# doubiliu/bellman-mpc

Measured on AMD Instinct MI355X. Metric: Groth16 constraints/sec, BLS12-381, 2^22-constraint R1CS, higher is better.
Workload: dtype u32 limbs (BLS12-381 Fp/Fr modular integer)

## Files before the change

bellman-mpc_amd/csrc/msm.h:

```cpp
#pragma once
#include <hip/hip_runtime.h>
#include <stddef.h>
#include <stdint.h>

#include <mutex>

#include "curve.cuh"
#include "kinfo.h"

namespace bh {

constexpr uint32_t G1_TABLE_REC = 32;

struct MsmShape {
  int c;
  int W;
  int NB;
  int L;
  int S;
  int Wb;
  int pre;
  int rec;
  uint32_t bk_lo = 0, bk_hi = 0;
  bool bucket_shard() const { return bk_hi > bk_lo; }
  uint32_t red_lo() const { return bucket_shard() ? bk_lo : 0u; }
  uint32_t red_nb() const { return bucket_shard() ? bk_hi - bk_lo : (uint32_t)NB; }
};
constexpr uint32_t BUCKET_SHARD_GRANULE = 1024;
MsmShape msm_shape(size_t n, int c_override);
int msm_table_c(size_t n);
MsmShape msm_shape_table(size_t n, int c);

uint32_t reduce_block_max(bool g2);
inline uint32_t reduce_threads_for(uint32_t nbr, uint32_t L, bool g2) {
  const uint32_t T = nbr / L, bmax = reduce_block_max(g2);
  return T < bmax ? T : bmax;
}
inline uint32_t reduce_block_threads(const MsmShape& sh, bool g2) {
  return reduce_threads_for((uint32_t)sh.NB, (uint32_t)sh.L, g2);
}
inline int reduce_lg2(uint32_t x) {
  int r = 0;
  while ((1u << r) < x) r++;
  return r;
}
inline int reduce_shift_for(uint32_t nbr, uint32_t L, bool g2) {
  return reduce_lg2(L) + reduce_lg2(reduce_threads_for(nbr, L, g2));
}
inline int reduce_split_shift(const MsmShape& sh, bool g2) {
  return sh.Wb == 1 ? reduce_shift_for(sh.red_nb(), (uint32_t)sh.L, g2) : -1;
}
inline void reduce_level2(uint32_t nblk, bool g2, uint32_t* BT2, uint32_t* Lb) {
  const uint32_t bmax = g2 ? 128u : 256u;
  uint32_t lb = 1;
  while ((size_t)bmax * lb < nblk) lb <<= 1;
  uint32_t t = 1;
  while ((size_t)t * lb < nblk) t <<= 1;
  *BT2 = t;
  *Lb = lb;
}

struct MsmTiming {
  hipEvent_t ev_acc_begin = nullptr, ev_acc_end = nullptr;
};

constexpr uint32_t G2_TABLE_REC = 64;

template <class C>
struct MsmWorkspace {
  size_t cap_n = 0, cap_E = 0, cap_nbt = 0, cap_segs = 0, cap_T = 0;
  uint32_t *entries = nullptr, *counts = nullptr, *offsets = nullptr, *cursor = nullptr, *scan_scratch = nullptr,
           *cont_bucket = nullptr, *tilecounts = nullptr, *tscan = nullptr;
  uint2* recs = nullptr;
  size_t cap_tc = 0;
  typename C::P *bucket_sums = nullptr, *conts = nullptr, *seg_weighted = nullptr, *seg_sum = nullptr,
                *window_sums = nullptr;
// ... 21 lines not shown
template <class C>
hipError_t msm_accumulate(MsmWorkspace<C>& ws, hipStream_t st, const uint32_t* d_bases, size_t n, const MsmShape& sh,
                          MsmTiming* timing);
template <class C>
hipError_t msm_front(MsmWorkspace<C>& ws, hipStream_t st, const uint32_t* d_bases, const uint32_t* d_scalars,
                     size_t n, const int32_t* d_idx, uint32_t base_offset, const MsmShape& sh, MsmTiming* timing);
template <class C>
hipError_t msm_back(MsmWorkspace<C>& ws, hipStream_t st, size_t n, const MsmShape& sh, typename C::P* host_out,
                    int max_span = -1, hipEvent_t acc_done = nullptr, const uint32_t* d_span_words = nullptr);

size_t scan_scratch_words(size_t n);
template <class C>
void msm_acc_kernels(std::vector<KernInfo>& v);
template <class C>
void msm_back_kernels(std::vector<KernInfo>& v);
size_t reduce_blocks_resident_per_cu_g1();
constexpr uint32_t MAX_SPAN_BLOCKS = 256;
inline uint32_t max_span_blocks(size_t nbt) {
  const size_t g = (nbt + 255) / 256;
  return (uint32_t)(g < 1 ? 1 : (g > MAX_SPAN_BLOCKS ? MAX_SPAN_BLOCKS : g));
}
inline uint32_t max_span_host(const uint32_t* h_words, size_t nbt) {
  uint32_t m = 0;
  for (uint32_t b = 0, g = max_span_blocks(nbt); b < g; b++) m = h_words[b] > m ? h_words[b] : m;
  return m;
}
hipError_t max_span(const uint32_t* counts, const uint32_t* offsets, size_t nbt, uint32_t S, uint32_t* d_words,
                    uint32_t* h_words, hipStream_t st);
void exclusive_scan(const uint32_t* in, uint32_t* out, size_t n, uint32_t* scratch, hipStream_t st);
hipError_t scalars_prepare(const uint32_t* d_in, uint32_t* d_out, size_t n, int mode, int log_perm, hipStream_t st);
hipError_t density_index(const uint64_t* d_words, size_t n, uint32_t base_offset, int32_t* d_idx, uint32_t* d_tmp,
// ... 16 lines not shown
```

bellman-mpc_amd/csrc/msm_common.hip:

```cpp
#include "msm.h"

#include <algorithm>

namespace bh {

static inline unsigned blocks_for(size_t n, unsigned bs) { return (unsigned)((n + bs - 1) / bs); }


__device__ __forceinline__ size_t scan_len(size_t n, const uint32_t* dn) {
  return dn ? min(n, (size_t)*dn + 1) : n;
}
__global__ void __launch_bounds__(256) k_scan_tile(const uint32_t* in, uint32_t* out, uint32_t* tile_sums, size_t n,
                                                   const uint32_t* dn) {
  __shared__ uint32_t s[256];
  n = scan_len(n, dn);
  if ((size_t)blockIdx.x * 1024 >= n) {
    if (threadIdx.x == 0 && tile_sums) tile_sums[blockIdx.x] = 0;
    return;
  }
  const size_t base = (size_t)blockIdx.x * 1024 + threadIdx.x * 4;
  uint32_t v[4];
  uint32_t local = 0;
#pragma unroll
  for (int i = 0; i < 4; i++) {
// ... 132 lines not shown
  if (d > half) {
    carry = 1;
    return (int)d - (int)(1u << c);
  }
  carry = 0;
  return (int)d;
}

__device__ __forceinline__ void load_scalar(const uint32_t* scalars, size_t i, uint32_t* s) {
  const uint4* p = reinterpret_cast<const uint4*>(scalars + i * 8);
  uint4 a = p[0], b = p[1];
  s[0] = a.x; s[1] = a.y; s[2] = a.z; s[3] = a.w;
  s[4] = b.x; s[5] = b.y; s[6] = b.z; s[7] = b.w;
}

static constexpr size_t REDUCE_T_MIN = 16384;

MsmShape msm_shape(size_t n, int c_override) {
  MsmShape sh;
  int c = c_override;
  if (c <= 0) {
    int lg = 0;
    while (((size_t)1 << (lg + 1)) <= n) lg++;
    int c0 = std::max(4, std::min(16, lg - 6));
    int best = c0, best_fill = -1;
    for (int cc = std::max(4, c0 - 1); cc <= std::min(16, c0 + 1); cc++) {
      const int W = (256 + cc - 1) / cc;
      const int top = 256 - (W - 1) * cc;
      const int fill = top * 16 / cc;
      if (fill > best_fill || (fill == best_fill && cc == c0)) { best = cc; best_fill = fill; }
    }
    c = best;
  }
  sh.c = c;
  sh.W = (256 + c - 1) / c;
  sh.NB = 1 << (c - 1);
  sh.L = std::min<int>(8, sh.NB);
  while (sh.L > 1 && (size_t)sh.W * (size_t)(sh.NB / sh.L) < REDUCE_T_MIN) sh.L >>= 1;
  size_t E = n * (size_t)sh.W;
  int S = 16;
  while (S < 256 && E / (size_t)(2 * S) >= ((size_t)1 << 18)) S <<= 1;
  sh.S = S;
  sh.Wb = sh.W;
  sh.pre = 0;
  sh.rec = 0;
  return sh;
}

uint32_t reduce_block_max(bool g2) { return g2 ? 128u : 256u; }

size_t seg_entries(size_t n, size_t used, int W) {
  (void)used;
  return std::max<size_t>(n, 1) * (size_t)std::max(W, 1);
// ... 3 lines not shown
  int best = 16;
  double best_cost = 1e300;
  for (int c = 8; c <= 24; c++) {
    const int W = (256 + c - 1) / c;
    if (255 - (W - 1) * c < 10) continue;
    const double cost = (double)n * W + 6.5 * (double)((size_t)1 << (c - 1));
    if (cost < best_cost) { best_cost = cost; best = c; }
  }
  return best;
}

MsmShape msm_shape_table(size_t n, int c) {
  MsmShape sh = msm_shape(n, c);
  sh.Wb = 1;
  sh.pre = 1;
  while (sh.L > 1 && (size_t)(sh.NB / sh.L) < REDUCE_T_MIN) sh.L >>= 1;
  return sh;
}

static constexpr int PT_TILE = 4096;

__global__ void __launch_bounds__(256) k_part_count(const uint32_t* scalars, size_t n, const int32_t* idx,
                                                    DigitCfg cfg, int lo_bits, uint32_t P, uint32_t ntiles,
                                                    uint32_t plo, uint32_t phi, uint32_t* tilecounts) {
  extern __shared__ uint32_t hist[];
  for (uint32_t i = threadIdx.x; i < P; i += 256) hist[i] = 0;
  __syncthreads();
  const size_t s0 = (size_t)blockIdx.x * PT_TILE;
  const size_t s1 = min(s0 + PT_TILE, n);
  for (size_t s = s0 + threadIdx.x; s < s1; s += 256) {
    if (idx && idx[s] < 0) continue;
// ... 232 lines not shown
  return e;
}

hipError_t density_index(const uint64_t* d_words, size_t n, uint32_t base_offset, int32_t* d_idx, uint32_t* d_tmp,
                         uint32_t* d_scan_scratch, hipStream_t st) {
  const size_t nwords = (n + 63) / 64;
  if (nwords == 0) return hipSuccess;
  hipLaunchKernelGGL(k_density_popc, dim3(blocks_for(nwords, 256)), dim3(256), 0, st, d_words, nwords, d_tmp);
  exclusive_scan(d_tmp, d_tmp, nwords, d_scan_scratch, st);
  hipLaunchKernelGGL(k_density_index, dim3(blocks_for(n, 256)), dim3(256), 0, st, d_words, d_tmp, n, base_offset,
                     d_idx);
  return hipGetLastError();
}

}
```

bellman-mpc_amd/csrc/msm_g1_back.hip:

```cpp
#include "msm_impl.cuh"

namespace bh {
extern template struct MsmWorkspace<G1Ops>;
extern template void fit_segments<G1Ops>(MsmShape&, size_t);
extern template void fit_segments_E<G1Ops>(MsmShape&, size_t);
extern template hipError_t msm_sort<G1Ops>(MsmWorkspace<G1Ops>&, hipStream_t, const uint32_t*, size_t, const int32_t*,
                                            uint32_t, const MsmShape&);
extern template hipError_t msm_accumulate<G1Ops>(MsmWorkspace<G1Ops>&, hipStream_t, const uint32_t*, size_t,
                                                  const MsmShape&, MsmTiming*);

template hipError_t msm_window_sums<G1Ops>(MsmWorkspace<G1Ops>&, hipStream_t, const uint32_t*, const uint32_t*, size_t,
                                         const int32_t*, uint32_t, const MsmShape&, MsmTiming*);
template hipError_t msm_front<G1Ops>(MsmWorkspace<G1Ops>&, hipStream_t, const uint32_t*, const uint32_t*, size_t,
                                   const int32_t*, uint32_t, const MsmShape&, MsmTiming*);
template hipError_t msm_back<G1Ops>(MsmWorkspace<G1Ops>&, hipStream_t, size_t, const MsmShape&, typename G1Ops::P*, int, hipEvent_t, const uint32_t*);
template void msm_back_kernels<G1Ops>(std::vector<KernInfo>&);

size_t reduce_blocks_resident_per_cu_g1() {
  int blocks = 1;
  const int BT = (int)reduce_block_max(false);
  if (hipOccupancyMaxActiveBlocksPerMultiprocessor(&blocks, (const void*)k_reduce_blocks<G1Ops>, BT,
                                                   BT * sizeof(typename G1Ops::P)) != hipSuccess ||
      blocks < 1)
    blocks = 1;
  return (size_t)blocks * BT;
}
}
```

bellman-mpc_amd/csrc/msm_impl.cuh:

```cuda
#pragma once
#include <cstdlib>

#include "msm.h"
#include <algorithm>


namespace bh {

static inline unsigned msm_blocks_for(size_t n, unsigned bs) { return (unsigned)((n + bs - 1) / bs); }

template <class C>
__device__ __forceinline__ void store_point(typename C::P* dst, const typename C::P& p) {
  constexpr int WORDS = sizeof(typename C::P) / 16;
  const uint4* s = reinterpret_cast<const uint4*>(&p);
  uint4* d = reinterpret_cast<uint4*>(dst);
#pragma unroll
  for (int k = 0; k < WORDS; k++) d[k] = s[k];
}
template <class C>
__device__ __forceinline__ typename C::P load_point(const typename C::P* src) {
  typename C::P p;
  constexpr int WORDS = sizeof(typename C::P) / 16;
  const uint4* s = reinterpret_cast<const uint4*>(src);
  uint4* d = reinterpret_cast<uint4*>(&p);
// ... 149 lines not shown
      if (tid == 0) store_point<C>(&conts[s_first + 1], acc);
      __syncthreads();
    }
  }
}


template <class C>
__device__ __forceinline__ typename C::P dbl_times(typename C::P v, int k) {
  for (int j = 0; j < k; j++) v = C::dbl(v);
  return v;
}

template <class C>
__device__ __forceinline__ void block_epilogue(typename C::P v, const typename C::P& base, int lg1,
                                               const typename C::P& extra, int lg2, bool split, typename C::P* lds,
                                               typename C::P* s_blk) {
  const uint32_t i = threadIdx.x, BT = blockDim.x;
  int lgBT = 0;
  while ((1u << lgBT) < BT) lgBT++;
  const int n_final = lg2 >= 0 ? 2 : 1;
  store_point<C>(&lds[i], v);
  __syncthreads();
  const int steps = 2 * lgBT + n_final;
  for (int st = 0; st < steps; st++) {
    typename C::P a = v, b;
    bool act;
    uint32_t dst = i;
    if (st < lgBT) {
      const uint32_t d = 1u << st;
      act = i + d < BT;
      if (act) b = load_point<C>(&lds[i + d]);
    } else if (st < lgBT + n_final) {
      const bool first = st == lgBT;
      if (first) {
        b = i + 1 < BT ? load_point<C>(&lds[i + 1]) : C::identity();
        if (i == 0) *s_blk = load_point<C>(&lds[0]);
      } else {
        b = v;
      }
      b = dbl_times<C>(b, first ? lg1 : lg2);
      a = first ? base : extra;
      act = true;
    } else {
      const uint32_t h = BT >> (st - lgBT - n_final + 1);
      act = split ? i < 2 * h : i < h;
      if (act) {
        dst = i < h ? i : BT + (i - h);
        a = load_point<C>(&lds[dst]);
        b = load_point<C>(&lds[dst + h]);
      }
    }
    __syncthreads();
    if (act) {
      v = C::add(a, b);
      store_point<C>(&lds[dst], v);
    }
    if (split && st == lgBT + n_final - 1) store_point<C>(&lds[BT + i], extra);
    __syncthreads();
  }
}

template <class C>
__global__ void __launch_bounds__(256) k_reduce_blocks(const uint32_t* counts, const uint32_t* offsets,
                                                       const typename C::P* bucket_sums, const typename C::P* conts,
                                                       uint32_t S, uint32_t b0, uint32_t NB, uint32_t L, int lgL,
                                                       uint32_t nblk, int fold, typename C::P* Y, typename C::P* Ssum,
                                                       const uint32_t* span_words, uint32_t span_g, uint32_t fold_span) {
  extern __shared__ uint4 lds_raw[];
  typename C::P* lds = reinterpret_cast<typename C::P*>(lds_raw);
  if (span_words) fold = block_span(span_words, span_g) <= fold_span ? 1 : 0;
  const uint32_t i = threadIdx.x;
  const uint32_t w = blockIdx.x / nblk, blk = blockIdx.x % nblk;
  const uint32_t gb0 = b0 + w * NB + (blk * blockDim.x + i) * L;
  constexpr bool acc_lds = sizeof(typename C::P) > 256;
  typename C::P run = C::identity(), acc = C::identity(), bk = C::identity();
  if (acc_lds) store_point<C>(&lds[i], acc);
  int k = (int)L - 1;
  uint32_t op = 0, c_next = 0, c_end = 0;
  while (k >= 0) {
    typename C::P a, b;
    if (op == 0) {
      const uint32_t gb = gb0 + (uint32_t)k, cnt = counts[gb];
      bk = C::identity();
      c_next = c_end = 0;
      if (cnt) {
        bk = load_point<C>(&bucket_sums[gb]);
        const uint32_t off = offsets[gb];
        const uint32_t s_first = off / S, s_last = (off + cnt - 1) / S;
        c_next = s_first + 1;
        c_end = s_last > s_first ? (fold ? s_last + 1 : s_first + 2) : c_next;
      }
      op = c_next < c_end ? 1 : 2;
      continue;
    }
    if (op == 1) { a = bk; b = load_point<C>(&conts[c_next]); }
    else if (op == 2) { a = run; b = bk; }
    else { a = acc_lds ? load_point<C>(&lds[i]) : acc; b = run; }
    const typename C::P r = C::add(a, b);
    if (op == 1) {
      bk = r;
      if (++c_next == c_end) op = 2;
    } else if (op == 2) {
      run = r;
      op = 3;
    } else {
      if (acc_lds) store_point<C>(&lds[i], r);
      else acc = r;
      op = 0;
      k--;
    }
  }
  if (acc_lds) acc = load_point<C>(&lds[i]);
  __syncthreads();
  typename C::P s_blk;
  block_epilogue<C>(run, acc, lgL, acc, -1, false, lds, &s_blk);
  if (i == 0) {
    store_point<C>(&Y[blockIdx.x], load_point<C>(&lds[0]));
    store_point<C>(&Ssum[blockIdx.x], s_blk);
  }
}

template <class C>
__global__ void __launch_bounds__(256) k_reduce_window(const typename C::P* Y, const typename C::P* Ssum,
                                                       uint32_t nblk, uint32_t Lb, int lgLb, int lgM, int split,
                                                       typename C::P* out) {
  extern __shared__ uint4 lds_raw[];
  typename C::P* lds = reinterpret_cast<typename C::P*>(lds_raw);
  const uint32_t i = threadIdx.x, w = blockIdx.x;
  const size_t base = (size_t)w * nblk + (size_t)i * Lb;
  typename C::P run = C::identity(), acc = C::identity(), p = C::identity();
  for (uint32_t it = 0; it < 3 * Lb; it++) {
    const uint32_t k = Lb - 1 - it / 3, op = it % 3;
    const bool in = i * Lb + k < nblk;
    typename C::P a, b;
    if (op == 0) { a = acc; b = run; }
    else if (op == 1) { a = run; b = in ? load_point<C>(&Ssum[base + k]) : C::identity(); }
    else { a = p; b = in ? load_point<C>(&Y[base + k]) : C::identity(); }
    const typename C::P r = C::add(a, b);
    if (op == 0) acc = r;
    else if (op == 1) run = r;
    else p = r;
  }
  typename C::P s_all;
  block_epilogue<C>(run, acc, lgLb, p, split ? -1 : lgM, split != 0, lds, &s_all);
  if (i == 0) {
    if (split) {
      out[0] = C::reduce(load_point<C>(&lds[blockDim.x]));
      out[1] = C::reduce(load_point<C>(&lds[0]));
      out[2] = C::reduce(s_all);
    } else {
      out[w] = C::reduce(load_point<C>(&lds[0]));
    }
  }
}

#define G2_SB() __builtin_amdgcn_sched_barrier(0)
template <class F, int NW, int NQ, bool ZZ_LDS, bool DIRECT = false, class Issue>
__device__ __forceinline__ void accumulate_lds(uint4 (*pre)[64], int lane, int nq, bool limbs,
                                               const uint32_t* entries, const uint32_t* offsets, uint32_t start,
                                               uint32_t end, uint32_t pos0, uint32_t seg, uint32_t b, uint32_t next,
                                               bool started_here, uint32_t e_cur, uint32_t e_next, Issue& issue,
                                               XYZZ<F>* bucket_sums, XYZZ<F>* conts,
                                               const uint32_t* bases = nullptr, uint32_t rec = 0) {
  using T = typename F::T;
  using Cv = CurveOps<F>;
  constexpr int VW = (NW % 4 == 0) ? 4 : 2;
  constexpr int RH = NW / VW;
// ... 311 lines not shown
    if (hipOccupancyMaxActiveBlocksPerMultiprocessor(&blocks, k, 256, 0) != hipSuccess || blocks < 1) blocks = 1;
    return (size_t)cus * (size_t)blocks * 256;
  }();
  constexpr size_t ROUNDS = 3, MIN_S = 8;
  const size_t slots = std::max<size_t>(ROUNDS * conc / 256 * 256, 256);
  size_t S = (E + slots - 1) / slots;
  sh.S = (int)std::min<size_t>(std::max<size_t>(S, MIN_S), (size_t)1 << 16);
}

template <class C>
size_t MsmWorkspace<C>::bytes_needed(size_t n) {
  MsmShape sh = msm_shape(n, 0);
  size_t E = n * (size_t)sh.W;
  size_t nbt = (size_t)sh.Wb * sh.NB;
  size_t segs = (E + sh.S - 1) / sh.S + 1;
  size_t T = (size_t)sh.Wb * (sh.NB / sh.L);
  return E * 4 + nbt * 4 * 3 + 16 + nbt * sizeof(typename C::P) + segs * sizeof(typename C::P) +
         2 * T * sizeof(typename C::P) + n * 4;
}

template <class C>
hipError_t MsmWorkspace<C>::grow(size_t E, size_t nbt, size_t segs, size_t T) {
  hipError_t err;
  if (E > cap_E) {
    if (entries) hipFree(entries);
    if (recs) hipFree(recs);
    entries = nullptr;
    recs = nullptr;
    if ((err = hipMalloc(&entries, std::max<size_t>(E, 1) * 4)) != hipSuccess) return err;
    if ((err = hipMalloc(&recs, std::max<size_t>(E, 1) * 8)) != hipSuccess) return err;
    cap_E = E;
// ... 31 lines not shown
    cap_T = T;
  }
  if (!window_sums) {
    if ((err = hipMalloc(&window_sums, 256 * sizeof(typename C::P))) != hipSuccess) return err;
    if ((err = hipHostMalloc(&host_window_sums, 256 * sizeof(typename C::P), hipHostMallocDefault)) != hipSuccess)
      return err;
  }
  return hipSuccess;
}

template <class C>
hipError_t MsmWorkspace<C>::reserve_shape(size_t n, const MsmShape& sh) {
  const size_t E = n * (size_t)sh.W;
  const size_t nbt = (size_t)sh.Wb * sh.NB;
  const size_t segs = (E + sh.S - 1) / sh.S + 1;
  const size_t T = (size_t)sh.Wb * (sh.NB / sh.L);
  const size_t tc = sort_tilecount_words(sh, n);
  if (tc > cap_tc) {
    if (tilecounts) hipFree(tilecounts);
    if (tscan) hipFree(tscan);
    tilecounts = tscan = nullptr;
    hipError_t err;
    if ((err = hipMalloc(&tilecounts, tc * 4)) != hipSuccess) return err;
    if ((err = hipMalloc(&tscan, scan_scratch_words(tc) * 4 + 64)) != hipSuccess) return err;
    cap_tc = tc;
  }
  return grow(E, nbt, segs, T);
}

template <class C>
hipError_t MsmWorkspace<C>::reserve(size_t n_max) {
// ... 93 lines not shown
};

struct AccView {
  const uint32_t *counts, *offsets;
  uint32_t S;
  size_t E;
  const uint32_t* span_words;
};
template <class C>
AccView acc_view(const MsmWorkspace<C>& ws, size_t n, const MsmShape& sh) {
  return AccView{ws.counts, ws.offsets, (uint32_t)sh.S, n * (size_t)sh.W, nullptr};
}

template <class C>
static void reduce_range(MsmWorkspace<C>& ws, const AccView& v, hipStream_t st, const MsmShape& sh, size_t segs,
                         size_t span, bool fold, bool seq, uint32_t b0, uint32_t nbr, uint32_t L, uint32_t y_off,
                         typename C::P* out, const SpanSrc& dev = SpanSrc()) {
  constexpr bool G2 = sizeof(typename C::P) > 256;
  const size_t nb_all = (size_t)sh.Wb * nbr;
  const size_t nbt = (size_t)sh.Wb * sh.NB;
  if (dev.words || (!fold && seq)) {
    constexpr int Q = 4;
    constexpr uint32_t B = G2 ? 128 : 256;
    if (dev.words || span >= 2)
      hipLaunchKernelGGL((k_cont_seq<C, Q>), dim3(msm_blocks_for(nb_all * Q, B)), dim3(B), B * sizeof(typename C::P),
                         st, v.counts, v.offsets, b0, (uint32_t)nb_all, v.S, ws.conts, dev.words, dev.g,
                         dev.fold_span, dev.seq_max);
    if (dev.words)
      hipLaunchKernelGGL((k_cont_long<C>), dim3(std::min<unsigned>(msm_blocks_for(nb_all, B), 256u)), dim3(B),
                         B * sizeof(typename C::P), st, v.counts, v.offsets, b0, (uint32_t)nb_all, v.S, ws.conts,
                         dev.words, dev.g, dev.seq_max);
  } else if (!fold) {
    for (size_t stride = 1; stride < span; stride *= 4)
      hipLaunchKernelGGL((k_cont_treeF<C, 4>), dim3(msm_blocks_for(segs, 256)), dim3(256), 0, st, ws.cont_bucket,
                         v.counts, v.offsets, (uint32_t)nbt, v.S, (uint32_t)stride, b0, (uint32_t)(b0 + nb_all),
                         ws.conts);
  }
  const uint32_t T = nbr / L;
  const uint32_t BT = reduce_threads_for(nbr, L, G2);
  const uint32_t nblk = T / BT;
  uint32_t BT2, Lb;
  reduce_level2(nblk, G2, &BT2, &Lb);
  const int split = sh.Wb == 1 ? 1 : 0;
  hipLaunchKernelGGL(k_reduce_blocks<C>, dim3((unsigned)(sh.Wb * nblk)), dim3(BT), BT * sizeof(typename C::P), st,
                     v.counts, v.offsets, ws.bucket_sums, ws.conts, v.S, b0, (uint32_t)sh.NB, L, reduce_lg2(L), nblk,
                     fold ? 1 : 0, ws.seg_weighted + y_off, ws.seg_sum + y_off, dev.words, dev.g, dev.fold_span);
  hipLaunchKernelGGL(k_reduce_window<C>, dim3((unsigned)sh.Wb), dim3(BT2), 2 * BT2 * sizeof(typename C::P), st,
                     ws.seg_weighted + y_off, ws.seg_sum + y_off, nblk, Lb, reduce_lg2(Lb),
                     reduce_lg2(L) + reduce_lg2(BT), split, out);
}

template <class C>
hipError_t msm_back(MsmWorkspace<C>& ws, hipStream_t st, size_t n, const MsmShape& sh, typename C::P* host_out,
                    int max_span, hipEvent_t acc_done, const uint32_t* d_span_words) {
  constexpr size_t REDUCE_FOLD_SPAN = 8;
  const AccView v = acc_view<C>(ws, n, sh);
  const size_t segs = (v.E + v.S - 1) / v.S;
  const size_t span = max_span >= 0 ? (size_t)max_span : segs;
  const bool fold = max_span >= 0 && span <= REDUCE_FOLD_SPAN;
  const bool seq = max_span >= 0 && span <= cont_seq_max();
  SpanSrc dev;
  if (max_span < 0 && d_span_words) {
    dev.words = d_span_words;
    dev.g = max_span_blocks((size_t)sh.Wb * sh.red_nb());
    dev.fold_span = (uint32_t)REDUCE_FOLD_SPAN;
    dev.seq_max = (uint32_t)cont_seq_max();
  }
  (void)acc_done;
  reduce_range<C>(ws, v, st, sh, segs, span, fold, seq, sh.red_lo(), sh.red_nb(), (uint32_t)sh.L, 0, ws.window_sums,
                  dev);
  const int outs = sh.bucket_shard() ? 3 : (sh.Wb == 1 ? 2 : sh.Wb);
  hipMemcpyAsync(host_out, ws.window_sums, outs * sizeof(typename C::P), hipMemcpyDeviceToHost, st);
  return hipGetLastError();
}

template <class C>
void msm_acc_kernels(std::vector<KernInfo>& v) {
  v.push_back({std::is_same<C, G1Ops>::value ? "k_accumulate_pf<G1>" : "k_accumulate_pf<G2>",
               (const void*)k_accumulate_pf<C>, 256, 0});
  if constexpr (!std::is_same<C, G1Ops>::value)
    v.push_back({"k_accumulate_g2d", (const void*)k_accumulate_g2d<C>, 256, 0});
}
template <class C>
void msm_back_kernels(std::vector<KernInfo>& v) {
  constexpr bool G2 = sizeof(typename C::P) > 256;
  const size_t P = sizeof(typename C::P);
  const int B = G2 ? 128 : 256, BT = (int)reduce_block_max(G2);
  v.push_back({G2 ? "k_reduce_blocks<G2>" : "k_reduce_blocks<G1>", (const void*)k_reduce_blocks<C>, BT, BT * P});
  v.push_back({G2 ? "k_reduce_window<G2>" : "k_reduce_window<G1>", (const void*)k_reduce_window<C>, BT,
               2 * BT * P});
  v.push_back({G2 ? "k_cont_seq<G2>" : "k_cont_seq<G1>", (const void*)k_cont_seq<C, 4>, B, B * P});
  v.push_back({G2 ? "k_cont_long<G2>" : "k_cont_long<G1>", (const void*)k_cont_long<C>, B, B * P});
  v.push_back({G2 ? "k_cont_treeF<G2>" : "k_cont_treeF<G1>", (const void*)k_cont_treeF<C, 4>, 256, 0});
}

template <class C>
hipError_t msm_window_sums(MsmWorkspace<C>& ws, hipStream_t st, const uint32_t* d_bases, const uint32_t* d_scalars,
                           size_t n, const int32_t* d_idx, uint32_t base_offset, const MsmShape& sh,
                           MsmTiming* timing) {
  hipError_t e = msm_front<C>(ws, st, d_bases, d_scalars, n, d_idx, base_offset, sh, timing);
  if (e != hipSuccess) return e;
  e = ws.reserve_shape(n, sh);
  if (e != hipSuccess) return e;
  return msm_back<C>(ws, st, n, sh, ws.host_window_sums);
}

}
```

bellman-mpc_amd/csrc/prover.hip:

```cpp
#include <stdio.h>
#include <string.h>

#include <algorithm>
#include <chrono>
#include <condition_variable>
#include <cstdlib>
#include <thread>

#include "api_internal.h"
#include "crs.h"
#include "dist_h.h"

using namespace bh;

namespace {

struct Reader {
  const uint8_t* p;
  const uint8_t* end;
  bool take(size_t n, const uint8_t** out) {
    if ((size_t)(end - p) < n) return false;
    *out = p;
    p += n;
    return true;
// ... 627 lines not shown
  auto full = [&](bh_srs* v, size_t used) {
    return ensure_table(ctx, v, table_c_for(used / (v == &params->h ? N : Naux)), 0, v->n);
  };
  if ((s = full(&params->h, m - 1))) return s;
  if ((s = full(&params->l, na))) return s;
  if ((s = full(&params->a, a_aux_used))) return s;
  if ((s = full(&params->b_g1, b_aux_used))) return s;
  return full(&params->b_g2, b_aux_used);
}

bool prover_serial() {
  const char* e = getenv("BH_PROVER_SERIAL");
  return e && e[0] == '1';
}

size_t reduce_resident_threads(bh_ctx* ctx, bool full) {
  static const size_t per_cu = reduce_blocks_resident_per_cu_g1();
  static std::once_flag once[64];
  static int ncu[64];
  const int d = ctx->device & 63;
  std::call_once(once[d], [&] {
    if (hipDeviceGetAttribute(&ncu[d], hipDeviceAttributeMultiprocessorCount, ctx->device) != hipSuccess) ncu[d] = 1;
  });
  const int cus = full ? ncu[d] : std::max(1, ncu[d] / 4);
  return per_cu * (size_t)std::max(cus, 1);
}


struct LaneHooks {
  std::function<void()> after_accs, before_tails, after_tails;
};
thread_local LaneHooks t_lane;

bh_status compute_msms(bh_ctx* ctx, const bh_params* params, const bh_witness* w, size_t shard, size_t nshards,
                       Jac<Fp> res1[6], Jac<bh::Fp2> res2[2], Exchanger* ex = nullptr, bool may_build = true,
                       UploadSync* up = nullptr) {
  const auto t0 = std::chrono::steady_clock::now();
  if (bh_status sc = scratch_check(ctx)) return sc;
  bh_params* mparams = const_cast<bh_params*>(params);
  std::shared_lock<std::shared_mutex> prd(mparams->mu, std::defer_lock);
  struct DrainOnError {
    bh_ctx* c;
// ... 126 lines not shown
    his[j] = jobs[j].hi;
    if (his[j] == los[j]) continue;
    const bh_srs* srs = jobs[j].srs;
    use_table[j] = jobs[j].table_c && srs->win_covers(jobs[j].table_c, jobs[j].blo, jobs[j].bhi);
    if (jobs[j].bk_hi && !use_table[j]) {
      fprintf(stderr, "bellman_hip: bucket shard without its window table (HBM short): set BH_SHARD_BUCKETS=0\n");
      return BH_ERR_OUT_OF_MEMORY;
    }
    shapes[j] = use_table[j] ? msm_shape_table(his[j] - los[j], srs->win_c)
                             : msm_shape(his[j] - los[j], ctx->window_override);
    if (use_table[j]) shapes[j].rec = srs->win_rec;
    if (jobs[j].bk_hi) {
      MsmShape& sh = shapes[j];
      sh.bk_lo = jobs[j].bk_lo;
      sh.bk_hi = jobs[j].bk_hi;
      const uint32_t BT = reduce_block_max(jobs[j].g2);
      while (sh.L > 1 && ((uint32_t)sh.L * BT > BUCKET_SHARD_GRANULE || sh.red_nb() / (uint32_t)sh.L < 16384u))
        sh.L >>= 1;
      const double f = bucket_cdf(sh.c, sh.W, sh.bk_hi) - bucket_cdf(sh.c, sh.W, sh.bk_lo);
      const size_t E = std::max<size_t>((size_t)((double)jobs[j].used * f), 1);
      if (jobs[j].g2) fit_segments_E<G2Ops>(sh, E);
      else fit_segments_E<G1Ops>(sh, E);
    } else {
      const size_t nj = his[j] - los[j];
      const size_t used_j = (size_t)((unsigned __int128)jobs[j].used * nj / std::max<size_t>(jobs[j].n, 1));
      const size_t E = seg_entries(nj, used_j, shapes[j].W);
      if (jobs[j].g2) fit_segments_E<G2Ops>(shapes[j], E);
      else fit_segments_E<G1Ops>(shapes[j], E);
    }
    if (jobs[j].table_c) n_large++;
    if (use_table[j]) n_table++;
  }
  auto enqueue_h = [&](hipEvent_t after) -> bh_status {
// ... 145 lines not shown
    return BH_OK;
  };
  BH_TRY_HIP(hipEventRecord(jev[33], sS));
  if (!(up && up->on_vector)) BH_TRY_HIP(hipStreamWaitEvent(sH, jev[33], 0));
  int big[8], nbig = 0, small[8], nsmall = 0;
  hipStream_t acc_stream[8] = {};
  for (int j = 0; j < 8; j++) {
    const size_t n = his[j] - los[j];
    if (!n || (host_in && j >= 5)) continue;
    if (n < SMALL_JOB && !jobs[j].is_h) small[nsmall++] = j;
    else big[nbig++] = j;
  }
  int h_pos = nbig;
  for (int q = 0; q < nbig; q++)
    if (jobs[big[q]].is_h) h_pos = q;
  if (nbig > 0) {
    MsmShape& sl = shapes[big[nbig - 1]];
    const int last_threads =
        last_full ? (int)std::min<size_t>(reduce_resident_threads(ctx, true), 1 << 20) : 65536;
    const int nb = (int)sl.red_nb();
    int L = sl.L;
    while (L > 1 && (size_t)sl.Wb * (size_t)(nb / L) < (size_t)last_threads) L >>= 1;
    sl.L = L;
  }
  bool h_late = up != nullptr;
  BH_TRY_HIP(hipStreamWaitEvent(sT, jev[33], 0));
  auto run_small = [&]() -> bh_status {
    for (int i = 0; i < nsmall; i++) {
      bh_status e = sort_job(small[i], sT);
      if (!e) e = acc_job(small[i], sT);
      if (!e) e = tail_job(small[i], sT);
      if (e) return e;
    }
    return BH_OK;
  };
  auto sort_h_or = [&](int j) -> bh_status {
    if (!jobs[j].is_h) return sort_job(j, sS);
    if (!dh) return sort_job(j, sH);
    BH_TRY_HIP(hipStreamWaitEvent(sS, ctx->ev[1], 0));
// ... 796 lines not shown
```

Baseline: 77.89 million.

## Replace bucket running-sum reduction with row/column decomposition

Replaces the per-thread L-bucket running-sum reduction (k_reduce_blocks + k_reduce_window) with a 2D row/column scheme. Buckets are viewed as an R x Cn grid, column sums and row sums are built via multi-level tree kernels, and a final kernel combines them with a doubling by lc. Continuation folding is split out into its own k_cont_fold kernel. This removes the serial per-thread L-length chains and the occupancy-based L tuning, in exchange for more kernel launches and extra partial-point memory traffic.

Result: faster. 81.40 million (median of 6 runs) (+4.5%).

```diff
diff --git a/bellman-mpc_amd/csrc/msm.h b/bellman-mpc_amd/csrc/msm.h
--- a/bellman-mpc_amd/csrc/msm.h
+++ b/bellman-mpc_amd/csrc/msm.h
@@ -7,6 +7,7 @@
 
 #include "curve.cuh"
 #include "kinfo.h"
+#include "msm_rowcol.h"
 
 namespace bh {
 
@@ -16,7 +17,6 @@
   int c;
   int W;
   int NB;
-  int L;
   int S;
   int Wb;
   int pre;
@@ -32,34 +32,18 @@
 MsmShape msm_shape_table(size_t n, int c);
 
 uint32_t reduce_block_max(bool g2);
-inline uint32_t reduce_threads_for(uint32_t nbr, uint32_t L, bool g2) {
-  const uint32_t T = nbr / L, bmax = reduce_block_max(g2);
-  return T < bmax ? T : bmax;
-}
-inline uint32_t reduce_block_threads(const MsmShape& sh, bool g2) {
-  return reduce_threads_for((uint32_t)sh.NB, (uint32_t)sh.L, g2);
-}
 inline int reduce_lg2(uint32_t x) {
   int r = 0;
   while ((1u << r) < x) r++;
   return r;
 }
-inline int reduce_shift_for(uint32_t nbr, uint32_t L, bool g2) {
-  return reduce_lg2(L) + reduce_lg2(reduce_threads_for(nbr, L, g2));
+inline int reduce_split_shift(const MsmShape& sh, bool g2) {
+  return sh.Wb == 1 ? rowcol_geom(sh.red_nb(), ROWCOL_QLG, g2).lc : -1;
 }
-inline int reduce_split_shift(const MsmShape& sh, bool g2) {
-  return sh.Wb == 1 ? reduce_shift_for(sh.red_nb(), (uint32_t)sh.L, g2) : -1;
+inline size_t reduce_partial_points(const MsmShape& sh, bool g2) {
+  const RowColGeom g = rowcol_geom(sh.red_nb(), ROWCOL_QLG, g2);
+  return (size_t)sh.Wb * (g.col_points > g.row_points ? g.col_points : g.row_points);
 }
-inline void reduce_level2(uint32_t nblk, bool g2, uint32_t* BT2, uint32_t* Lb) {
-  const uint32_t bmax = g2 ? 128u : 256u;
-  uint32_t lb = 1;
-  while ((size_t)bmax * lb < nblk) lb <<= 1;
-  uint32_t t = 1;
-  while ((size_t)t * lb < nblk) t <<= 1;
-  *BT2 = t;
-  *Lb = lb;
-}
-
 struct MsmTiming {
   hipEvent_t ev_acc_begin = nullptr, ev_acc_end = nullptr;
 };
@@ -111,7 +95,6 @@
 void msm_acc_kernels(std::vector<KernInfo>& v);
 template <class C>
 void msm_back_kernels(std::vector<KernInfo>& v);
-size_t reduce_blocks_resident_per_cu_g1();
 constexpr uint32_t MAX_SPAN_BLOCKS = 256;
 inline uint32_t max_span_blocks(size_t nbt) {
   const size_t g = (nbt + 255) / 256;
diff --git a/bellman-mpc_amd/csrc/msm_common.hip b/bellman-mpc_amd/csrc/msm_common.hip
--- a/bellman-mpc_amd/csrc/msm_common.hip
+++ b/bellman-mpc_amd/csrc/msm_common.hip
@@ -170,8 +170,6 @@
   s[4] = b.x; s[5] = b.y; s[6] = b.z; s[7] = b.w;
 }
 
-static constexpr size_t REDUCE_T_MIN = 16384;
-
 MsmShape msm_shape(size_t n, int c_override) {
   MsmShape sh;
   int c = c_override;
@@ -191,8 +189,6 @@
   sh.c = c;
   sh.W = (256 + c - 1) / c;
   sh.NB = 1 << (c - 1);
-  sh.L = std::min<int>(8, sh.NB);
-  while (sh.L > 1 && (size_t)sh.W * (size_t)(sh.NB / sh.L) < REDUCE_T_MIN) sh.L >>= 1;
   size_t E = n * (size_t)sh.W;
   int S = 16;
   while (S < 256 && E / (size_t)(2 * S) >= ((size_t)1 << 18)) S <<= 1;
@@ -226,7 +222,6 @@
   MsmShape sh = msm_shape(n, c);
   sh.Wb = 1;
   sh.pre = 1;
-  while (sh.L > 1 && (size_t)(sh.NB / sh.L) < REDUCE_T_MIN) sh.L >>= 1;
   return sh;
 }
 
@@ -489,3 +484,18 @@
 }
 
 }
+
+extern "C" int bh_selftest_rowcol_geometry(uint32_t nbr, int qlg, int g2, uint64_t* out, size_t cap) {
+  const bh::RowColGeom g = bh::rowcol_geom(nbr, qlg, g2 != 0);
+  const size_t need = 9 + 5 * (size_t)(g.ncol + g.nrow);
+  if (!out || cap < need) return -1;
+  size_t k = 0;
+  out[k++] = (uint64_t)g.lc; out[k++] = g.Cn; out[k++] = g.R; out[k++] = (uint64_t)g.ncol; out[k++] = (uint64_t)g.nrow;
+  out[k++] = g.final_threads; out[k++] = g.final_per_thread; out[k++] = g.col_points; out[k++] = g.row_points;
+  for (int r = 0; r < 2; r++)
+    for (int i = 0; i < (r ? g.nrow : g.ncol); i++) {
+      const bh::RowColLevel& l = r ? g.row[i] : g.col[i];
+      out[k++] = l.rows_in; out[k++] = l.rows_out; out[k++] = l.inner; out[k++] = l.Q; out[k++] = l.out_off;
+    }
+  return (int)k;
+}
diff --git a/bellman-mpc_amd/csrc/msm_g1_back.hip b/bellman-mpc_amd/csrc/msm_g1_back.hip
--- a/bellman-mpc_amd/csrc/msm_g1_back.hip
+++ b/bellman-mpc_amd/csrc/msm_g1_back.hip
@@ -15,14 +15,4 @@
                                    const int32_t*, uint32_t, const MsmShape&, MsmTiming*);
 template hipError_t msm_back<G1Ops>(MsmWorkspace<G1Ops>&, hipStream_t, size_t, const MsmShape&, typename G1Ops::P*, int, hipEvent_t, const uint32_t*);
 template void msm_back_kernels<G1Ops>(std::vector<KernInfo>&);
-
-size_t reduce_blocks_resident_per_cu_g1() {
-  int blocks = 1;
-  const int BT = (int)reduce_block_max(false);
-  if (hipOccupancyMaxActiveBlocksPerMultiprocessor(&blocks, (const void*)k_reduce_blocks<G1Ops>, BT,
-                                                   BT * sizeof(typename G1Ops::P)) != hipSuccess ||
-      blocks < 1)
-    blocks = 1;
-  return (size_t)blocks * BT;
 }
-}
diff --git a/bellman-mpc_amd/csrc/msm_impl.cuh b/bellman-mpc_amd/csrc/msm_impl.cuh
--- a/bellman-mpc_amd/csrc/msm_impl.cuh
+++ b/bellman-mpc_amd/csrc/msm_impl.cuh
@@ -187,144 +187,136 @@
 
 template <class C>
 __device__ __forceinline__ void block_epilogue(typename C::P v, const typename C::P& base, int lg1,
-                                               const typename C::P& extra, int lg2, bool split, typename C::P* lds,
-                                               typename C::P* s_blk) {
+                                               typename C::P* lds, typename C::P* s_blk) {
   const uint32_t i = threadIdx.x, BT = blockDim.x;
   int lgBT = 0;
   while ((1u << lgBT) < BT) lgBT++;
-  const int n_final = lg2 >= 0 ? 2 : 1;
   store_point<C>(&lds[i], v);
   __syncthreads();
-  const int steps = 2 * lgBT + n_final;
+  const int steps = 2 * lgBT + 1;
   for (int st = 0; st < steps; st++) {
     typename C::P a = v, b;
     bool act;
-    uint32_t dst = i;
     if (st < lgBT) {
       const uint32_t d = 1u << st;
       act = i + d < BT;
       if (act) b = load_point<C>(&lds[i + d]);
-    } else if (st < lgBT + n_final) {
-      const bool first = st == lgBT;
-      if (first) {
-        b = i + 1 < BT ? load_point<C>(&lds[i + 1]) : C::identity();
-        if (i == 0) *s_blk = load_point<C>(&lds[0]);
-      } else {
-        b = v;
-      }
-      b = dbl_times<C>(b, first ? lg1 : lg2);
-      a = first ? base : extra;
+    } else if (st == lgBT) {
+      b = i + 1 < BT ? load_point<C>(&lds[i + 1]) : C::identity();
+      if (i == 0) *s_blk = load_point<C>(&lds[0]);
+      b = dbl_times<C>(b, lg1);
+      a = base;
       act = true;
     } else {
-      const uint32_t h = BT >> (st - lgBT - n_final + 1);
-      act = split ? i < 2 * h : i < h;
+      const uint32_t h = BT >> (st - lgBT);
+      act = i < h;
       if (act) {
-        dst = i < h ? i : BT + (i - h);
-        a = load_point<C>(&lds[dst]);
-        b = load_point<C>(&lds[dst + h]);
+        a = load_point<C>(&lds[i]);
+        b = load_point<C>(&lds[i + h]);
       }
     }
     __syncthreads();
     if (act) {
       v = C::add(a, b);
-      store_point<C>(&lds[dst], v);
-    }
-    if (split && st == lgBT + n_final - 1) store_point<C>(&lds[BT + i], extra);
+      store_point<C>(&lds[i], v);
+    }
     __syncthreads();
   }
 }
 
-template <class C>
-__global__ void __launch_bounds__(256) k_reduce_blocks(const uint32_t* counts, const uint32_t* offsets,
-                                                       const typename C::P* bucket_sums, const typename C::P* conts,
-                                                       uint32_t S, uint32_t b0, uint32_t NB, uint32_t L, int lgL,
-                                                       uint32_t nblk, int fold, typename C::P* Y, typename C::P* Ssum,
-                                                       const uint32_t* span_words, uint32_t span_g, uint32_t fold_span) {
+
+template <class C>
+__global__ void __launch_bounds__(256) k_cont_fold(const uint32_t* cont_bucket, const uint32_t* counts,
+                                                   const uint32_t* offsets, uint32_t S, uint32_t b_lo, uint32_t b_hi,
+                                                   int fold, const typename C::P* conts, typename C::P* bucket_sums,
+                                                   const uint32_t* span_words, uint32_t span_g, uint32_t fold_span) {
+  const uint32_t E_lo = offsets[b_lo], E_hi = offsets[b_hi];
+  const size_t per = (size_t)blockDim.x * S;
+  const size_t run_first = E_lo / per, run_end = (E_hi + per - 1) / per;
+  if (E_hi <= E_lo || run_first + blockIdx.x >= run_end) return;
+  if (span_words) fold = block_span(span_words, span_g) <= fold_span ? 1 : 0;
+  for (size_t run = run_first + blockIdx.x; run < run_end; run += gridDim.x) {
+    const uint32_t s = (uint32_t)(run * blockDim.x + threadIdx.x);
+    const size_t pos0 = (size_t)s * S;
+    if (pos0 < E_lo || pos0 >= E_hi) continue;
+    const uint32_t b = cont_bucket[s];
+    if (b == 0xffffffffu) continue;
+    const uint32_t off = offsets[b];
+    const uint32_t s_first = off / S;
+    if (s != s_first + 1) continue;
+    const uint32_t n = fold ? (off + counts[b] - 1) / S - s_first : 1u;
+    typename C::P v = load_point<C>(&bucket_sums[b]);
+    for (uint32_t i = 0; i < n; i++) v = C::add(v, load_point<C>(&conts[s + i]));
+    store_point<C>(&bucket_sums[b], v);
+  }
+}
+constexpr unsigned CONT_FOLD_BLOCKS = 512;
+
+template <class C>
+struct SumJob {
+  const typename C::P* in = nullptr;
+  typename C::P* out = nullptr;
+  const uint32_t* counts = nullptr;
+  uint32_t rows_in = 0, inner = 1, Q = 1, n_out = 0, blocks = 0;
+};
+template <class C>
+__global__ void __launch_bounds__(256) k_rowcol_sum(SumJob<C> a, SumJob<C> b) {
+  const bool second = blockIdx.x >= a.blocks;
+  const SumJob<C> J = second ? b : a;
+  const uint32_t i = (blockIdx.x - (second ? a.blocks : 0u)) * blockDim.x + threadIdx.x;
+  if (i >= J.n_out) return;
+  const uint32_t g = i / J.inner, j = i - g * J.inner;
+  const uint32_t r_end = min(g * J.Q + J.Q, J.rows_in);
+  typename C::P acc = C::identity();
+  for (uint32_t r = g * J.Q; r < r_end; r++) {
+    const size_t e = (size_t)r * J.inner + j;
+    if (J.counts && J.counts[e] == 0) continue;
+    acc = C::add(acc, load_point<C>(&J.in[e]));
+  }
+  store_point<C>(&J.out[i], acc);
+}
+
+template <class C>
+__global__ void __launch_bounds__(256) k_rowcol_final(const typename C::P* col, uint32_t Cn, const typename C::P* row,
+                                                      uint32_t R, uint32_t Lb, int lgLb, int lc, typename C::P* out) {
   extern __shared__ uint4 lds_raw[];
   typename C::P* lds = reinterpret_cast<typename C::P*>(lds_raw);
-  if (span_words) fold = block_span(span_words, span_g) <= fold_span ? 1 : 0;
   const uint32_t i = threadIdx.x;
-  const uint32_t w = blockIdx.x / nblk, blk = blockIdx.x % nblk;
-  const uint32_t gb0 = b0 + w * NB + (blk * blockDim.x + i) * L;
-  constexpr bool acc_lds = sizeof(typename C::P) > 256;
-  typename C::P run = C::identity(), acc = C::identity(), bk = C::identity();
-  if (acc_lds) store_point<C>(&lds[i], acc);
-  int k = (int)L - 1;
-  uint32_t op = 0, c_next = 0, c_end = 0;
-  while (k >= 0) {
-    typename C::P a, b;
-    if (op == 0) {
-      const uint32_t gb = gb0 + (uint32_t)k, cnt = counts[gb];
-      bk = C::identity();
-      c_next = c_end = 0;
-      if (cnt) {
-        bk = load_point<C>(&bucket_sums[gb]);
-        const uint32_t off = offsets[gb];
-        const uint32_t s_first = off / S, s_last = (off + cnt - 1) / S;
-        c_next = s_first + 1;
-        c_end = s_last > s_first ? (fold ? s_last + 1 : s_first + 2) : c_next;
-      }
-      op = c_next < c_end ? 1 : 2;
-      continue;
-    }
-    if (op == 1) { a = bk; b = load_point<C>(&conts[c_next]); }
-    else if (op == 2) { a = run; b = bk; }
-    else { a = acc_lds ? load_point<C>(&lds[i]) : acc; b = run; }
-    const typename C::P r = C::add(a, b);
-    if (op == 1) {
-      bk = r;
-      if (++c_next == c_end) op = 2;
-    } else if (op == 2) {
-      run = r;
-      op = 3;
-    } else {
-      if (acc_lds) store_point<C>(&lds[i], r);
+  const bool split = lc < 0;
+  const uint32_t w = split ? 0u : blockIdx.x;
+  const int p_first = split ? (blockIdx.x == 1 ? 0 : 1) : 0, p_last = split ? p_first : 1;
+#pragma unroll 1
+  for (int pass = p_first; pass <= p_last; pass++) {
+    const bool rows = pass == 0;
+    const typename C::P* in = rows ? row + (size_t)w * R : col + (size_t)w * Cn;
+    const uint32_t n = rows ? R : Cn;
+    typename C::P run = C::identity(), acc = C::identity();
+    if (!split && !rows && i == 0) acc = load_point<C>(&out[w]);
+    for (uint32_t it = 0; it < 2 * Lb; it++) {
+      const uint32_t k = Lb - 1 - it / 2;
+      const bool to_run = ((it & 1u) != 0) == rows;
+      typename C::P a, b;
+      if (to_run) { a = run; b = i * Lb + k < n ? load_point<C>(&in[i * Lb + k]) : C::identity(); }
+      else { a = acc; b = run; }
+      const typename C::P r = C::add(a, b);
+      if (to_run) run = r;
       else acc = r;
-      op = 0;
-      k--;
-    }
-  }
-  if (acc_lds) acc = load_point<C>(&lds[i]);
-  __syncthreads();
-  typename C::P s_blk;
-  block_epilogue<C>(run, acc, lgL, acc, -1, false, lds, &s_blk);
-  if (i == 0) {
-    store_point<C>(&Y[blockIdx.x], load_point<C>(&lds[0]));
-    store_point<C>(&Ssum[blockIdx.x], s_blk);
-  }
-}
-
-template <class C>
-__global__ void __launch_bounds__(256) k_reduce_window(const typename C::P* Y, const typename C::P* Ssum,
-                                                       uint32_t nblk, uint32_t Lb, int lgLb, int lgM, int split,
-                                                       typename C::P* out) {
-  extern __shared__ uint4 lds_raw[];
-  typename C::P* lds = reinterpret_cast<typename C::P*>(lds_raw);
-  const uint32_t i = threadIdx.x, w = blockIdx.x;
-  const size_t base = (size_t)w * nblk + (size_t)i * Lb;
-  typename C::P run = C::identity(), acc = C::identity(), p = C::identity();
-  for (uint32_t it = 0; it < 3 * Lb; it++) {
-    const uint32_t k = Lb - 1 - it / 3, op = it % 3;
-    const bool in = i * Lb + k < nblk;
-    typename C::P a, b;
-    if (op == 0) { a = acc; b = run; }
-    else if (op == 1) { a = run; b = in ? load_point<C>(&Ssum[base + k]) : C::identity(); }
-    else { a = p; b = in ? load_point<C>(&Y[base + k]) : C::identity(); }
-    const typename C::P r = C::add(a, b);
-    if (op == 0) acc = r;
-    else if (op == 1) run = r;
-    else p = r;
-  }
-  typename C::P s_all;
-  block_epilogue<C>(run, acc, lgLb, p, split ? -1 : lgM, split != 0, lds, &s_all);
-  if (i == 0) {
-    if (split) {
-      out[0] = C::reduce(load_point<C>(&lds[blockDim.x]));
-      out[1] = C::reduce(load_point<C>(&lds[0]));
-      out[2] = C::reduce(s_all);
-    } else {
-      out[w] = C::reduce(load_point<C>(&lds[0]));
-    }
+    }
+    typename C::P s_all;
+    block_epilogue<C>(run, acc, lgLb, lds, &s_all);
+    if (i == 0) {
+      const typename C::P x = load_point<C>(&lds[0]);
+      if (!split) {
+        if (rows) store_point<C>(&out[w], dbl_times<C>(x, lc));
+        else out[w] = C::reduce(x);
+      } else if (rows) {
+        out[1] = C::reduce(x);
+        out[2] = C::reduce(s_all);
+      } else {
+        out[0] = C::reduce(x);
+      }
+    }
+    __syncthreads();
   }
 }
 
@@ -666,7 +658,7 @@
   size_t E = n * (size_t)sh.W;
   size_t nbt = (size_t)sh.Wb * sh.NB;
   size_t segs = (E + sh.S - 1) / sh.S + 1;
-  size_t T = (size_t)sh.Wb * (sh.NB / sh.L);
+  size_t T = reduce_partial_points(sh, sizeof(typename C::P) > 256);
   return E * 4 + nbt * 4 * 3 + 16 + nbt * sizeof(typename C::P) + segs * sizeof(typename C::P) +
          2 * T * sizeof(typename C::P) + n * 4;
 }
@@ -728,7 +720,7 @@
   const size_t E = n * (size_t)sh.W;
   const size_t nbt = (size_t)sh.Wb * sh.NB;
   const size_t segs = (E + sh.S - 1) / sh.S + 1;
-  const size_t T = (size_t)sh.Wb * (sh.NB / sh.L);
+  const size_t T = reduce_partial_points(sh, sizeof(typename C::P) > 256);
   const size_t tc = sort_tilecount_words(sh, n);
   if (tc > cap_tc) {
     if (tilecounts) hipFree(tilecounts);
@@ -852,7 +844,7 @@
 
 template <class C>
 static void reduce_range(MsmWorkspace<C>& ws, const AccView& v, hipStream_t st, const MsmShape& sh, size_t segs,
-                         size_t span, bool fold, bool seq, uint32_t b0, uint32_t nbr, uint32_t L, uint32_t y_off,
+                         size_t span, bool fold, bool seq, uint32_t b0, uint32_t nbr,
                          typename C::P* out, const SpanSrc& dev = SpanSrc()) {
   constexpr bool G2 = sizeof(typename C::P) > 256;
   const size_t nb_all = (size_t)sh.Wb * nbr;
@@ -874,18 +866,36 @@
                          v.counts, v.offsets, (uint32_t)nbt, v.S, (uint32_t)stride, b0, (uint32_t)(b0 + nb_all),
                          ws.conts);
   }
-  const uint32_t T = nbr / L;
-  const uint32_t BT = reduce_threads_for(nbr, L, G2);
-  const uint32_t nblk = T / BT;
-  uint32_t BT2, Lb;
-  reduce_level2(nblk, G2, &BT2, &Lb);
-  const int split = sh.Wb == 1 ? 1 : 0;
-  hipLaunchKernelGGL(k_reduce_blocks<C>, dim3((unsigned)(sh.Wb * nblk)), dim3(BT), BT * sizeof(typename C::P), st,
-                     v.counts, v.offsets, ws.bucket_sums, ws.conts, v.S, b0, (uint32_t)sh.NB, L, reduce_lg2(L), nblk,
-                     fold ? 1 : 0, ws.seg_weighted + y_off, ws.seg_sum + y_off, dev.words, dev.g, dev.fold_span);
-  hipLaunchKernelGGL(k_reduce_window<C>, dim3((unsigned)sh.Wb), dim3(BT2), 2 * BT2 * sizeof(typename C::P), st,
-                     ws.seg_weighted + y_off, ws.seg_sum + y_off, nblk, Lb, reduce_lg2(Lb),
-                     reduce_lg2(L) + reduce_lg2(BT), split, out);
+  const uint32_t Wb = (uint32_t)sh.Wb;
+  const unsigned fold_blocks = std::max(1u, std::min(msm_blocks_for(segs, 256), CONT_FOLD_BLOCKS));
+  hipLaunchKernelGGL(k_cont_fold<C>, dim3(fold_blocks), dim3(256), 0, st, ws.cont_bucket, v.counts, v.offsets, v.S,
+                     b0, (uint32_t)(b0 + nb_all), fold ? 1 : 0, ws.conts, ws.bucket_sums, dev.words, dev.g,
+                     dev.fold_span);
+  const RowColGeom g = rowcol_geom(nbr, ROWCOL_QLG, G2);
+  const uint32_t B = G2 ? 128 : 256;
+  for (int lv = 0; lv < std::max(g.ncol, g.nrow); lv++) {
+    SumJob<C> job[2];
+    for (int r = 0; r < 2; r++) {
+      if (lv >= (r ? g.nrow : g.ncol)) continue;
+      const RowColLevel* ls = r ? g.row : g.col;
+      typename C::P* part = r ? ws.seg_sum : ws.seg_weighted;
+      SumJob<C>& j = job[r];
+      j.in = lv ? part + (size_t)Wb * ls[lv - 1].out_off : ws.bucket_sums + b0;
+      j.out = part + (size_t)Wb * ls[lv].out_off;
+      j.counts = lv ? nullptr : v.counts + b0;
+      j.rows_in = Wb * ls[lv].rows_in;
+      j.inner = ls[lv].inner;
+      j.Q = ls[lv].Q;
+      j.n_out = Wb * ls[lv].rows_out * ls[lv].inner;
+      j.blocks = msm_blocks_for(j.n_out, B);
+    }
+    hipLaunchKernelGGL(k_rowcol_sum<C>, dim3(job[0].blocks + job[1].blocks), dim3(B), 0, st, job[0], job[1]);
+  }
+  hipLaunchKernelGGL(k_rowcol_final<C>, dim3(Wb == 1 ? 2u : Wb), dim3(g.final_threads),
+                     g.final_threads * sizeof(typename C::P), st,
+                     ws.seg_weighted + (size_t)Wb * g.col[g.ncol - 1].out_off, g.Cn,
+                     ws.seg_sum + (size_t)Wb * g.row[g.nrow - 1].out_off, g.R, g.final_per_thread,
+                     reduce_lg2(g.final_per_thread), Wb == 1 ? -1 : g.lc, out);
 }
 
 template <class C>
@@ -905,7 +915,7 @@
     dev.seq_max = (uint32_t)cont_seq_max();
   }
   (void)acc_done;
-  reduce_range<C>(ws, v, st, sh, segs, span, fold, seq, sh.red_lo(), sh.red_nb(), (uint32_t)sh.L, 0, ws.window_sums,
+  reduce_range<C>(ws, v, st, sh, segs, span, fold, seq, sh.red_lo(), sh.red_nb(), ws.window_sums,
                   dev);
   const int outs = sh.bucket_shard() ? 3 : (sh.Wb == 1 ? 2 : sh.Wb);
   hipMemcpyAsync(host_out, ws.window_sums, outs * sizeof(typename C::P), hipMemcpyDeviceToHost, st);
@@ -924,12 +934,12 @@
   constexpr bool G2 = sizeof(typename C::P) > 256;
   const size_t P = sizeof(typename C::P);
   const int B = G2 ? 128 : 256, BT = (int)reduce_block_max(G2);
-  v.push_back({G2 ? "k_reduce_blocks<G2>" : "k_reduce_blocks<G1>", (const void*)k_reduce_blocks<C>, BT, BT * P});
-  v.push_back({G2 ? "k_reduce_window<G2>" : "k_reduce_window<G1>", (const void*)k_reduce_window<C>, BT,
-               2 * BT * P});
   v.push_back({G2 ? "k_cont_seq<G2>" : "k_cont_seq<G1>", (const void*)k_cont_seq<C, 4>, B, B * P});
   v.push_back({G2 ? "k_cont_long<G2>" : "k_cont_long<G1>", (const void*)k_cont_long<C>, B, B * P});
   v.push_back({G2 ? "k_cont_treeF<G2>" : "k_cont_treeF<G1>", (const void*)k_cont_treeF<C, 4>, 256, 0});
+  v.push_back({G2 ? "k_cont_fold<G2>" : "k_cont_fold<G1>", (const void*)k_cont_fold<C>, 256, 0});
+  v.push_back({G2 ? "k_rowcol_sum<G2>" : "k_rowcol_sum<G1>", (const void*)k_rowcol_sum<C>, B, 0});
+  v.push_back({G2 ? "k_rowcol_final<G2>" : "k_rowcol_final<G1>", (const void*)k_rowcol_final<C>, BT, BT * P});
 }
 
 template <class C>
diff --git a/bellman-mpc_amd/csrc/msm_rowcol.h b/bellman-mpc_amd/csrc/msm_rowcol.h
--- /dev/null
+++ b/bellman-mpc_amd/csrc/msm_rowcol.h
@@ -0,0 +1,85 @@
+#pragma once
+#include <stddef.h>
+#include <stdint.h>
+
+namespace bh {
+
+constexpr int ROWCOL_MAX_LEVELS = 16;
+constexpr int ROWCOL_QLG = 3;
+constexpr int ROWCOL_MAX_LC = 10;
+
+struct RowColLevel {
+  uint32_t rows_in, rows_out, inner, Q;
+  size_t out_off;
+};
+
+struct RowColGeom {
+  int lc;
+  uint32_t Cn, R;
+  int ncol, nrow;
+  RowColLevel col[ROWCOL_MAX_LEVELS], row[ROWCOL_MAX_LEVELS];
+  size_t col_points, row_points;
+  uint32_t final_threads, final_per_thread;
+};
+
+inline int rowcol_lg2_ceil(uint32_t x) {
+  int r = 0;
+  while (((uint64_t)1 << r) < x) r++;
+  return r;
+}
+
+inline int rowcol_levels(uint32_t rows, uint32_t inner, int qlg, RowColLevel* lv, size_t* points) {
+  const int bits = rowcol_lg2_ceil(rows);
+  int n = (bits + qlg - 1) / qlg;
+  if (n < 1) n = 1;
+  size_t off = 0;
+  for (int i = 0; i < n; i++) {
+    const int b = bits / n + (i < bits % n ? 1 : 0);
+    lv[i].rows_in = rows;
+    lv[i].Q = 1u << b;
+    lv[i].rows_out = (rows + lv[i].Q - 1) / lv[i].Q;
+    lv[i].inner = inner;
+    lv[i].out_off = off;
+    off += (size_t)lv[i].rows_out * inner;
+    rows = lv[i].rows_out;
+  }
+  *points = off;
+  return n;
+}
+
+inline RowColGeom rowcol_geom(uint32_t nbr, int qlg, bool g2) {
+  RowColGeom g;
+  if (qlg < 2) qlg = 2;
+  int lc = (rowcol_lg2_ceil(nbr) + 1) / 2;
+  if (lc > ROWCOL_MAX_LC) lc = ROWCOL_MAX_LC;
+  g.lc = lc;
+  g.Cn = 1u << lc;
+  g.R = (nbr + g.Cn - 1) / g.Cn;
+  g.ncol = rowcol_levels(g.R, g.Cn, qlg, g.col, &g.col_points);
+  size_t off = 0;
+  const int bits = lc;
+  int n = (bits + qlg - 1) / qlg;
+  if (n < 1) n = 1;
+  uint32_t per_row = g.Cn;
+  for (int i = 0; i < n; i++) {
+    const int b = bits / n + (i < bits % n ? 1 : 0);
+    g.row[i].rows_in = g.R * per_row;
+    g.row[i].Q = 1u << b;
+    per_row >>= b;
+    g.row[i].rows_out = g.R * per_row;
+    g.row[i].inner = 1;
+    g.row[i].out_off = off;
+    off += g.row[i].rows_out;
+  }
+  g.nrow = n;
+  g.row_points = off;
+  const uint32_t m = g.Cn > g.R ? g.Cn : g.R, bmax = g2 ? 128u : 256u;
+  uint32_t lb = 1, t = 1;
+  while ((uint64_t)bmax * lb < m) lb <<= 1;
+  while ((uint64_t)t * lb < m) t <<= 1;
+  g.final_threads = t;
+  g.final_per_thread = lb;
+  return g;
+}
+
+}
diff --git a/bellman-mpc_amd/csrc/prover.hip b/bellman-mpc_amd/csrc/prover.hip
--- a/bellman-mpc_amd/csrc/prover.hip
+++ b/bellman-mpc_amd/csrc/prover.hip
@@ -665,18 +665,6 @@
   return e && e[0] == '1';
 }
 
-size_t reduce_resident_threads(bh_ctx* ctx, bool full) {
-  static const size_t per_cu = reduce_blocks_resident_per_cu_g1();
-  static std::once_flag once[64];
-  static int ncu[64];
-  const int d = ctx->device & 63;
-  std::call_once(once[d], [&] {
-    if (hipDeviceGetAttribute(&ncu[d], hipDeviceAttributeMultiprocessorCount, ctx->device) != hipSuccess) ncu[d] = 1;
-  });
-  const int cus = full ? ncu[d] : std::max(1, ncu[d] / 4);
-  return per_cu * (size_t)std::max(cus, 1);
-}
-
 
 struct LaneHooks {
   std::function<void()> after_accs, before_tails, after_tails;
@@ -833,9 +821,6 @@
       MsmShape& sh = shapes[j];
       sh.bk_lo = jobs[j].bk_lo;
       sh.bk_hi = jobs[j].bk_hi;
-      const uint32_t BT = reduce_block_max(jobs[j].g2);
-      while (sh.L > 1 && ((uint32_t)sh.L * BT > BUCKET_SHARD_GRANULE || sh.red_nb() / (uint32_t)sh.L < 16384u))
-        sh.L >>= 1;
       const double f = bucket_cdf(sh.c, sh.W, sh.bk_hi) - bucket_cdf(sh.c, sh.W, sh.bk_lo);
       const size_t E = std::max<size_t>((size_t)((double)jobs[j].used * f), 1);
       if (jobs[j].g2) fit_segments_E<G2Ops>(sh, E);
@@ -1011,15 +996,6 @@
   int h_pos = nbig;
   for (int q = 0; q < nbig; q++)
     if (jobs[big[q]].is_h) h_pos = q;
-  if (nbig > 0) {
-    MsmShape& sl = shapes[big[nbig - 1]];
-    const int last_threads =
-        last_full ? (int)std::min<size_t>(reduce_resident_threads(ctx, true), 1 << 20) : 65536;
-    const int nb = (int)sl.red_nb();
-    int L = sl.L;
-    while (L > 1 && (size_t)sl.Wb * (size_t)(nb / L) < (size_t)last_threads) L >>= 1;
-    sl.L = L;
-  }
   bool h_late = up != nullptr;
   BH_TRY_HIP(hipStreamWaitEvent(sT, jev[33], 0));
   auto run_small = [&]() -> bh_status {
```
